# michaelfeil/skyjo_rl

Measured on AMD Instinct MI355X. Metric: env-steps/sec (whole node) at 65 536 parallel 3-player games, higher is better.
Workload: dtype int8

## Files before the change

skyjo_rl_amd/csrc/skyjo_deal.h:

```cpp
#pragma once
#ifndef SKYJO_DEVICE_PARTS
#error "include skyjo_device.h"
#endif

__global__ void k_seed(SkParams P, const uint64_t *seeds, uint64_t base, int first, int count) {
  const int i = blockIdx.x * blockDim.x + threadIdx.x;
  if (i >= count) return;
  const int g = first + i;
  const uint64_t value = seeds ? seeds[i] : base + P.game_id0 + (uint64_t)g;
  const size_t G = (size_t)P.tiles * SK_TILE;
  P.seeds[g] = value;
  P.deals_consumed[g] = 0;
  for (int k = 0; k < SK_BANK; k++) P.spare_ready[(size_t)k * G + g] = 0;
  P.bank_head[g] = 0, P.busy[g] = 0, P.cancel[g] = 0, P.done_flag[g] = 0;
  if (P.rng_mode == SKYJO_RNG_MT19937) {
    uint32_t *mt = P.mt + (size_t)g * 624;
    uint32_t x = (uint32_t)(value + 1);
    mt[0] = x;
    for (int k = 1; k < 624; k++) {
      x = 1812433253u * (x ^ (x >> 30)) + (uint32_t)k;
      mt[k] = x;
    }
    P.mt_idx[g] = 0;
  }
// ... 385 lines not shown
      w |= (i < SK_NCARDS ? (uint32_t)((-2 + i / 10) & 0xff) : 0u) << (8 * j);
    }
    LW(pw + d) = w;
  }
#pragma unroll 1
  for (int seg = 0; seg < N + 2; seg++) {
    int base = pb, n = SK_NCARDS;
    if (seg == 1) {
      for (int p = 0; p < N; p++)
        for (int j = 0; j < 3; j++) LW((sk_pb(P.L, p) >> 2) + j) = LW(pw + 3 * p + j);
      for (int d = 0; d < (R + 3) / 4; d += 8) {
        uint32_t t[8];
#pragma unroll
        for (int k = 0; k < 8; k++) t[k] = LW(pw + 3 * N + d + k);
#pragma unroll
        for (int k = 0; k < 8; k++)
          if (d + k < (R + 3) / 4) LW(pw + d + k) = t[k];
      }
      n = R;
    } else if (seg >= 2) {
      const int p = seg - 2;
      for (int k = 0; k < 12; k++) LB(tmp + k) = (uint8_t)k, LB(sk_pb(P.L, p) + PB_VIS + k) = SKYJO_HAND_NONE;
      base = tmp, n = 12;
    }
    shuffle_lds(lp, base, n, r);
    if (seg >= 2) {
      const int p = seg - 2;
      int s0 = LB(tmp), s1 = LB(tmp + 1);
      const int blk = sk_pb(P.L, p);
      int c0 = LI(blk + PB_CARDS + s0), c1 = LI(blk + PB_CARDS + s1);
      LB(blk + PB_VIS + s0) = (uint8_t)c0, LB(blk + PB_VIS + s1) = (uint8_t)c1;
      LSH(blk + PB_SUM) = (int16_t)(c0 + c1);
      LB(blk + PB_HIDDEN) = 10;
      if (!P.L.indirect) LB(H_HIST + 2 + c0)++, LB(H_HIST + 2 + c1)++;
    }
  }
  for (int k = R; k < SK_NCARDS; k++) LB(pb + k) = 0;
  const int last = LI(pb + R - 1);
  LB(pb + R - 1) = 0;
  LB(pb + SK_NCARDS - 1) = (uint8_t)last;
  LB(H_HIST + 2 + last)++;
  int best = 0, bs = LSH(sk_pb(P.L, 0) + PB_SUM);
  for (int p = 1; p < N; p++) {
    int s = LSH(sk_pb(P.L, p) + PB_SUM);
    if (s > bs) bs = s, best = p;
  }
  LB(H_PHASE) = 0, LB(H_PLAYER) = (uint8_t)best, LB(H_FLAGS) = F_VALID, LB(H_STATUS) = SKYJO_ST_RESET;
  LB(H_NDRAW) = (uint8_t)(R - 1), LB(H_NDISC) = 1, LB(H_ROLE) = 0;
  LB(H_TOP) = (uint8_t)last, LB(H_HAND) = SKYJO_HAND_NONE;
  *(uint32_t *)(lp + LIDX(H_EPISODE)) = episode;
  refresh_minima(P, lp);
}

__device__ __forceinline__ bool deal_inline(const SkParams &P, uint8_t *lp, uint8_t *fp, int g, int tile, int lane, int head) {
  const uint32_t ep = P.deals_consumed[g];
  const int busy = P.busy[g];
  if (busy) {
    const bool cancelled = P.cancel[g] != 0;
    if (P.rng_mode == SKYJO_RNG_MT19937 && !cancelled) {
      const int w = wait_deal_done(P, g);
      if (w == SK_WAIT_TIMEOUT) {
        LB(H_FLAGS) = F_VALID | F_DONE, LB(H_STATUS) = SKYJO_ST_ERROR;
        for (int q = 0; q < P.L.N; q++) P.rewards[(size_t)g * P.L.N + q] = 0.0;
        return false;
      }
      P.cancel[g] = 1;
      if (w == SK_WAIT_OK) {
        load_spare(P, lp, busy - 1, tile, lane);
        bank_advance(P, lp, g, head, ep);
        return true;
      }
    }
    P.cancel[g] = 1;
  }
  if (P.rng_mode == SKYJO_RNG_MT19937) {
    MtStream<16> r;
    r.open(P.mt + (size_t)g * 624, P.mt_idx[g], fp);
    deal_into_lds(P, lp, r, ep);
    P.mt_idx[g] = r.close();
  } else {
    PhiloxStream r;
    r.open(P.seeds[g] + 1, ep, 0u, 0u);
    deal_into_lds(P, lp, r, ep);
  }
  LB(H_BANK) = (uint8_t)head;
  P.deals_consumed[g] = ep + 1;
  P.done[g] = 0;
  return true;
}

#define SK_SCAN_BLOCK 1024
__global__ __launch_bounds__(SK_SCAN_BLOCK) void k_scan(SkParams P, int list_sel) {
  __shared__ uint32_t wave_need[SK_SCAN_BLOCK / 64], block_first;
  const size_t G = (size_t)P.tiles * SK_TILE;
  const int lane = threadIdx.x & 63, wave = threadIdx.x >> 6;
  int32_t *list = P.deal_list + (size_t)list_sel * G;
  uint32_t *eps = P.deal_ep + (size_t)list_sel * G;
  for (int base = blockIdx.x * SK_SCAN_BLOCK; base < P.B; base += gridDim.x * SK_SCAN_BLOCK) {
    const int g = base + (int)threadIdx.x;
    bool need = false;
    int slot = 0, r = 0;
    uint32_t consumed = 0;
    if (g < P.B) {
      const uint8_t busy = P.busy[g];
      const int head = P.bank_head[g] % SK_BANK;
      consumed = P.deals_consumed[g];
      uint8_t ready[SK_BANK];
// ... 208 lines not shown
```

skyjo_rl_amd/csrc/skyjo_device.h:

```cpp
#pragma once
#include <hip/hip_runtime.h>
#include <stdint.h>

#include "../../include/skyjo_vec.h"
#include "skyjo_layout.h"
#include "skyjo_draw.h"

struct SkCounters {
  unsigned long long steps, episodes, illegal, resets, sum_len, reshuffles, iters, waits;
  double sum_score[SKYJO_MAX_PLAYERS];
  double sum_reward[SKYJO_MAX_PLAYERS];
  double sum_reward_sq[SKYJO_MAX_PLAYERS];
  double sum_refunded[SKYJO_MAX_PLAYERS];
};
#define SK_ERR_DEAL_TIMEOUT 1u
#ifndef SK_SCORE_EVERY
#define SK_SCORE_EVERY 32
#endif
#define SK_ACC_KINDS 4

#ifndef SK_BANK
#define SK_BANK 3
#endif

// ... 107 lines not shown

#define SK_DMA4(NT)                                                                                                     \
  asm volatile("s_mov_b32 %0, m0\n\ts_mov_b32 m0, %3\n\ts_nop 0\n\t"                                                    \
               "global_load_lds_dwordx4 %1, %2" NT "\n\tglobal_load_lds_dwordx4 %1, %2 offset:1024" NT "\n\t"           \
               "global_load_lds_dwordx4 %1, %2 offset:2048" NT "\n\tglobal_load_lds_dwordx4 %1, %2 offset:3072" NT "\n\t" \
               "s_mov_b32 m0, %0"                                                                                       \
               : "=&s"(keep)                                                                                            \
               : "v"(voff), "s"(base), "s"(lds)                                                                         \
               : "memory")
#define SK_DMA1(NT)                                                                                              \
  asm volatile("s_mov_b32 %0, m0\n\ts_mov_b32 m0, %3\n\ts_nop 0\n\tglobal_load_lds_dwordx4 %1, %2" NT "\n\ts_mov_b32 m0, %0" \
               : "=&s"(keep)                                                                                     \
               : "v"(voff), "s"(base), "s"(lds)                                                                  \
               : "memory")
template <bool NT>
__device__ __forceinline__ void dma_record(const uint8_t *base, uint32_t voff, uint32_t lds, int chunks) {
  uint32_t keep;
  int c = 0;
  for (; c + 4 <= chunks; c += 4) {
    if (NT) SK_DMA4(" nt");
    else SK_DMA4("");
    base += 4096, lds += 4096;
  }
  for (; c < chunks; c++) {
    if (NT) SK_DMA1(" nt");
    else SK_DMA1("");
    base += 1024, lds += 1024;
  }
}
#define SK_DMAB4(NT)                                                                                                        \
  asm volatile("s_mov_b32 %0, m0\n\ts_mov_b32 m0, %3\n\ts_nop 0\n\tglobal_load_lds_dwordx4 %1, %2" NT "\n\t"                \
               "s_add_u32 m0, m0, 0x3f0\n\ts_nop 0\n\tglobal_load_lds_dwordx4 %1, %2 offset:16" NT "\n\t"                   \
               "s_add_u32 m0, m0, 0x3f0\n\ts_nop 0\n\tglobal_load_lds_dwordx4 %1, %2 offset:32" NT "\n\t"                   \
               "s_add_u32 m0, m0, 0x3f0\n\ts_nop 0\n\tglobal_load_lds_dwordx4 %1, %2 offset:48" NT "\n\t"                   \
               "s_mov_b32 m0, %0"                                                                                           \
               : "=&s"(keep)                                                                                                \
               : "v"(voff), "s"(base), "s"(lds)                                                                             \
               : "memory", "scc")
template <bool NT>
__device__ __forceinline__ void dma_bank_record(const uint8_t *base, uint32_t voff, uint32_t lds, int chunks) {
  uint32_t keep;
  int c = 0;
  for (; c + 4 <= chunks; c += 4) {
    if (NT) SK_DMAB4(" nt");
    else SK_DMAB4("");
    base += 64, lds += 4096;
  }
  for (; c < chunks; c++) {
    if (NT) SK_DMA1(" nt");
    else SK_DMA1("");
    base += 16, lds += 1024;
  }
}
__device__ __forceinline__ void sk_vm_drain() { asm volatile("s_waitcnt vmcnt(0)" ::: "memory"); }

struct Stamps {
  unsigned long long t, acc[8];
};
#ifdef SK_STAMPS
#define STAMP_DECL Stamps st; st.t = __builtin_amdgcn_s_memtime(); for (int k_ = 0; k_ < 8; k_++) st.acc[k_] = 0
#define STAMP(i)                                                 \
  do {                                                           \
    __builtin_amdgcn_sched_barrier(0);                           \
    __builtin_amdgcn_s_waitcnt(0xc07f);  \
    unsigned long long st_n = __builtin_amdgcn_s_memtime();      \
    __builtin_amdgcn_s_waitcnt(0xc07f);                          \
    st.acc[i] += st_n - st.t;                                    \
    st.t = st_n;                                                 \
    __builtin_amdgcn_sched_barrier(0);                           \
  } while (0)
#define STAMP_STORE                                                        \
  do {                                                                     \
    if (lane == 0)                                                         \
      for (int k = 0; k < 8; k++) P.stamps[(size_t)tile * 8 + k] += st.acc[k]; \
  } while (0)
#else
#define STAMP_DECL Stamps st
#define STAMP(i)
#define STAMP_STORE
#endif
#ifdef SK_STAMPS_TOP
#define STAMP_N(n)
#define STAMP_T(t) STAMP(t)
#else
#define STAMP_N(n) STAMP(n)
#define STAMP_T(t)
#endif

#ifdef SK_TRACE
#define TRACE_DECL const unsigned long long trace_t0 = __builtin_amdgcn_s_memrealtime(), trace_c0 = __builtin_amdgcn_s_memtime(); unsigned long long trace_wait = 0, trace_w0 = 0
#define TRACE_WAIT_BEGIN trace_w0 = __builtin_amdgcn_s_memtime()
#define TRACE_WAIT_END trace_wait += __builtin_amdgcn_s_memtime() - trace_w0
#define TRACE_STORE(kind, tag, lane_, block_)                                                                    \
  do {                                                                                                           \
    if ((lane_) == 0) {                                                                                          \
      unsigned long long *tr = P.stamps + (((size_t)(2 * (kind) + ((tag) & 1u)) * P.tiles + (block_)) * 8);     \
      tr[0] = __builtin_amdgcn_s_getreg(63492);                                       \
      tr[1] = __builtin_amdgcn_s_getreg(63508);                                               \
      tr[2] = trace_t0, tr[3] = __builtin_amdgcn_s_memrealtime(), tr[4] = (tag);                                 \
      tr[5] = __builtin_amdgcn_s_memtime() - trace_c0;  \
      tr[6] = trace_wait;                        \
    }                                                                                                            \
  } while (0)
#else
#define TRACE_DECL
#define TRACE_WAIT_BEGIN
#define TRACE_WAIT_END
#define TRACE_STORE(kind, tag, lane_, block_)
#endif

#define SKYJO_DEVICE_PARTS 1
#include "skyjo_rng.h"
#include "skyjo_transition.h"
#include "skyjo_record.h"
#include "skyjo_step.h"
#include "skyjo_deal.h"
#include "skyjo_cycle.h"
#include "skyjo_callers.h"
```

skyjo_rl_amd/csrc/skyjo_record.h:

```cpp
#pragma once
#ifndef SKYJO_DEVICE_PARTS
#error "include skyjo_device.h"
#endif

template <bool INDIRECT>
__device__ __forceinline__ void emit_record(const SkParams &P, uint8_t *lp, const HdrRegs &h, const ObsRegs &ob, int action,
                                            uint8_t *out, uint4 *held = nullptr, const uint4 *pre_a = nullptr, uint32_t pre_b = 0) {
  const int phase = h.w0 & 0xff;
  const uint32_t q0 = ob.q0, q1 = ob.q1, q2 = ob.q2;
  const uint32_t act24 = ((uint32_t)action & 0xffu) << 24;
  uint32_t m[8];
  {
    const uint32_t pm = phase ? 0xffffffffu : 0u;
    m[0] = ob.nz0 & pm, m[1] = ob.nz1 & pm, m[2] = ob.nz2 & pm, m[3] = ob.hd0 & pm, m[4] = ob.hd1 & pm, m[5] = ob.hd2 & pm;
    m[6] = (phase ? 0u : 0x0101u) | (((h.w0 >> 8) & 0xffu) << 16) | ((uint32_t)phase << 24);
    m[7] = (((h.w0 >> 16) & F_DONE) ? 1u : 0u) | ((h.w0 >> 24) << 8) | ((h.w2 & 0xffffu) << 16);
  }
  const uint4 a = pre_a ? *pre_a : LQ(1);
  const uint32_t s8 = (pre_a ? pre_b : (uint32_t)LB(32)) | ((h.w1 >> 24) << 8) | ((h.w2 >> 24) << 16);
  if (INDIRECT) {
    uint4 *o = (uint4 *)out;
    uint4 b;
    b.x = s8 | (q0 << 24), b.y = (q0 >> 8) | (q1 << 24), b.z = (q1 >> 8) | (q2 << 24), b.w = (q2 >> 8) | act24;
    if (held) {
// ... 45 lines not shown
    uint4 v[6];
#pragma unroll
    for (int k = 0; k < 6; k++)
      if (c + k < n) v[k] = LQ(c + k);
#pragma unroll
    for (int k = 0; k < 6; k++)
      if (c + k < n) d[c + k] = v[k];
  }
}

__device__ __forceinline__ void bank_advance(const SkParams &P, uint8_t *lp, int g, int head, uint32_t dc) {
  const uint8_t nh = (uint8_t)((head + 1) % SK_BANK);
  P.bank_head[g] = nh;
  LB(H_BANK) = nh;
  P.deals_consumed[g] = dc + 1;
  P.done[g] = 0;
}

__device__ __forceinline__ bool consume_spare(const SkParams &P, uint8_t *lp, int tile, int lane, int g, int head) {
  const size_t G = (size_t)P.tiles * SK_TILE;
  const uint8_t ready = P.spare_ready[(size_t)head * G + g];
  const uint32_t dc = P.deals_consumed[g];
  if (!ready) return false;
  load_spare(P, lp, head, tile, lane);
  P.spare_ready[(size_t)head * G + g] = 0;
  bank_advance(P, lp, g, head, dc);
  return true;
}

struct SpareRegs {
  uint32_t dc;
  int head;
  uint8_t ready;
};
__device__ __forceinline__ void spare_issue(const SkParams &P, uint8_t *lp, uint32_t lds_tile, int tile, int lane, int g, SpareRegs &r) {
  const size_t G = (size_t)P.tiles * SK_TILE;
  r.head = LB(H_BANK) % SK_BANK;
  r.ready = P.spare_ready[(size_t)r.head * G + g];
  r.dc = P.deals_consumed[g];
  const uint32_t voff = (uint32_t)(bank_rec16(P, r.head, g) * 16);
  asm volatile("s_waitcnt lgkmcnt(0)" ::: "memory");
  dma_bank_record<false>((const uint8_t *)P.spare, voff, lds_tile, P.L.chunks);
}
__device__ __forceinline__ bool spare_commit(const SkParams &P, uint8_t *lp, int g, const SpareRegs &r) {
  sk_vm_drain();
  if (!r.ready) return false;
  P.spare_ready[(size_t)r.head * (size_t)P.tiles * SK_TILE + g] = 0;
  bank_advance(P, lp, g, r.head, r.dc);
  return true;
}

__device__ __forceinline__ constexpr int sk_stage_stride(int rec_bytes) { return ((rec_bytes >> 2) & 7) == 0 ? rec_bytes + 16 : rec_bytes; }

__device__ __forceinline__ bool deal_inline(const SkParams &P, uint8_t *lp, uint8_t *fp, int g, int tile, int lane, int head);
```

skyjo_rl_amd/csrc/skyjo_step.h:

```cpp
#pragma once
#ifndef SKYJO_DEVICE_PARTS
#error "include skyjo_device.h"
#endif

__device__ __forceinline__ void sk_publish_deals(const SkParams &P, int g) {
  const size_t G = (size_t)P.tiles * SK_TILE;
  const int b = P.busy[g];
  if (b) {
    const uint32_t tag = P.plan_tag[g];
    const uint32_t f = __hip_atomic_load(&P.done_flag[g], __ATOMIC_RELAXED, __HIP_MEMORY_SCOPE_AGENT);
    if ((f & 0x7fffffffu) == tag) {
      SK_FENCE_ACQUIRE(P);
      if (!P.cancel[g] && f == tag) P.spare_ready[(size_t)(b - 1) * G + g] = 1;
      P.busy[g] = 0, P.cancel[g] = 0;
    }
  }
}
__device__ __forceinline__ void sk_plan_deals(const SkParams &P, int g, int lane) {
  const size_t G = (size_t)P.tiles * SK_TILE;
  bool need = false, empty = false;
  if (g < P.B) {
    const uint8_t busy = P.busy[g];
    const int head = P.bank_head[g] % SK_BANK;
    const uint32_t consumed = P.deals_consumed[g];
// ... 32 lines not shown
__device__ __forceinline__ void sk_export_raw(const SkParams &P, uint8_t *lp, int g, uint8_t *o) {
  for (int c = 0; c < P.L.chunks; c++) ((uint4 *)o)[c] = LQ(c);
  double *d = (double *)(o + P.L.state_bytes);
  for (int p = 0; p < P.L.N; p++) d[p] = P.rewards[(size_t)g * P.L.N + p], d[P.L.N + p] = P.scores[(size_t)g * P.L.N + p];
  uint32_t *m = (uint32_t *)(d + 2 * P.L.N);
  m[0] = P.rng_mode == SKYJO_RNG_MT19937 ? (uint32_t)P.mt_idx[g] : 0u;
  m[1] = P.done[g];
}

__device__ __forceinline__ uint32_t sk_next_tag(uint32_t t) {
  t = (t + 1u) & 0x7fffffffu;
  return t ? t : 1u;
}
template <bool INDIRECT, bool POLICY, int NP, bool PLANAR = false>
__device__ __forceinline__ void step_body(const SkParams &Pin, const int tile, const int lane, uint32_t *lds_raw, const int32_t *actions,
                                          uint8_t *rec_out, int32_t *act_out, int iters, uint64_t policy_seed, uint64_t iter0,
                                          double *end_rew_out, uint8_t *end_out, uint8_t *raw_out, int raw_stride, const int cycle_len = 0,
                                          const bool defer_ok = true) {
  SkParams P = Pin;
  TRACE_DECL;
  if (NP > 0) P.L = sk_make_layout(NP, INDIRECT ? 1 : 0);
  const int g = tile * SK_TILE + lane;
  const uint32_t lds_tile = (uint32_t)(uintptr_t)(__attribute__((address_space(3))) uint32_t *)lds_raw;
  uint8_t *lp = (uint8_t *)lds_raw + lane * 16;
  uint8_t *stg = (uint8_t *)lds_raw + P.L.chunks * 1024;
  uint8_t *fp = stg + lane * 4;
  const int stg_bytes = (INDIRECT || PLANAR) ? 4096 : SK_TILE * (P.L.rec_bytes + 16);
  uint8_t *ap = stg + stg_bytes + lane * 8;
  constexpr bool DEFER = POLICY && NP > 0 && NP < 8;
  constexpr bool REGACC = NP > 0 && NP < 8;
  constexpr int NACC = REGACC ? SK_ACC_KINDS * NP : 1;
  double racc_store[NACC];
#pragma unroll
  for (int k = 0; k < NACC; k++) racc_store[k] = 0.0;
  double *racc = REGACC ? racc_store : nullptr;
  uint8_t *pendp = DEFER && defer_ok ? stg + stg_bytes + (REGACC ? 0 : SK_ACC_KINDS * P.L.N * 512) + lane * 16 : nullptr;
  int pend_fin = -1;
  if (!REGACC)
    for (int k = 0; k < SK_ACC_KINDS * P.L.N; k++) ACC(k) = 0.0;
  STAMP_DECL;
  if (!POLICY) tile_load(P, P.state, tile, lane, lp);
  else dma_record<true>((const uint8_t *)P.state, (uint32_t)((((size_t)tile * P.L.chunks) * SK_TILE + lane) * 16), lds_tile, P.L.chunks);
  if (P.ov_flags & 1u) sk_publish_deals(P, g);
  sk_vm_drain();
  HdrRegs h;
  HDR_LOAD(h);
  STAMP(0);
  const bool valid = ((h.w0 >> 16) & F_VALID) != 0;
  LaneCounters cnt;
  uint32_t r0 = 0, r1 = 0, r2 = 0, r3 = 0;
  const uint64_t gid = P.game_id0 + (uint64_t)g;
  ObsRegs ob;
  if (valid) obs_load(P, lp, (h.w0 >> 8) & 0xff, ob);
  for (int it = 0; it < iters; it++) {
    const uint64_t iter = iter0 + (uint64_t)it;
    if (POLICY && (it == 0 || (iter & 3) == 0)) {
      philox4x32_10((uint32_t)(iter >> 2), (uint32_t)gid, (uint32_t)(gid >> 32), 0x504F4C00u, (uint32_t)policy_seed,
                    (uint32_t)(policy_seed >> 32), r0, r1, r2, r3);
      for (int k = (int)(iter & 3); k > 0; k--) {
        const uint32_t t = r0;
        r0 = r1, r1 = r2, r2 = r3, r3 = t;
      }
    }
    STAMP_T(3);
    const uint32_t word = r0;
    if (POLICY) {
      r0 = r1, r1 = r2, r2 = r3, r3 = word;
    }
    int a = -1;
    if (valid) {
      const bool over = ((h.w0 >> 16) & F_DONE) != 0;
      if (!POLICY) a = actions[g];
      const bool skip = !POLICY && a == SKYJO_ACTION_SKIP;
      const bool acted = !over && !skip;
      SpareRegs sp;
      const bool resetting = over && P.auto_reset && !skip;
      if (resetting) spare_issue(P, lp, lds_tile, tile, lane, g, sp);
      STAMP_T(4);
      if (!over && !skip) {
        const uint32_t v0 = ob.q0, v1 = ob.q1, v2 = ob.q2;
        STAMP_N(2);
        const uint4 row_pre = LQ(sk_pb(P.L, (h.w0 >> 8) & 0xff) >> 4);
        asm volatile("" ::: "memory");
        if (POLICY) a = policy_pick(h.w0 & 0xff, ob, word);
#ifndef SK_STAMPS_FINE
        STAMP_N(3);
#endif
        apply_action<INDIRECT, NP, POLICY>(P, lp, fp, ap, h, v0, v1, v2, a, g, cnt, st, pendp, pend_fin, row_pre, racc);
#ifdef SK_STAMPS_FINE
        STAMP(6);
#else
        STAMP(5);
#endif
      } else if (!skip) {
        a = -1;
        if (P.auto_reset) {
          bool dealt = true;
          if (!spare_commit(P, lp, g, sp)) {
            dealt = deal_inline(P, lp, fp, g, tile, lane, sp.head);
            cnt.waits++;
          }
          HDR_LOAD(h);
          if (SK_OFTEN(dealt)) {
            h.w0 = (h.w0 & 0x00ffffffu) | ((uint32_t)SKYJO_ST_RESET << 24);
            cnt.resets++;
          }
        } else {
          h.w0 = (h.w0 & 0x00ffffffu) | ((uint32_t)SKYJO_ST_NOOP_DONE << 24);
        }
        STAMP(1);
      } else {
        a = -1;
      }
      if (!POLICY && acted && (unsigned)a >= (unsigned)SKYJO_NUM_ACTIONS) a = -2;
      if (!POLICY && end_out) {
        const bool end = acted && ((h.w0 >> 16) & F_DONE) != 0;
        end_out[g] = end ? 1 : 0;
        for (int q = 0; q < P.L.N; q++) end_rew_out[(size_t)g * P.L.N + q] = end ? P.rewards[(size_t)g * P.L.N + q] : 0.0;
      }
      const uint4 rec_a = LQ(1);
      const uint32_t rec_b = LB(32);
      const uint4 rec_row = LQ((sk_pb(P.L, (h.w0 >> 8) & 0xff) + PB_VIS) >> 4);
      asm volatile("" ::: "memory");
      obs_from_row(rec_row, ob);
      if (rec_out) {
        if (INDIRECT) {
          uint4 rr[4];
          emit_record<INDIRECT>(P, lp, h, ob, a, nullptr, rr, &rec_a, rec_b);
          if (PLANAR) {
            typedef uint32_t u32x4_t __attribute__((ext_vector_type(4)));
            uint8_t *blk = rec_out + ((size_t)it * P.tiles + (size_t)tile) * (SK_TILE * 64) + lane * 16;
#pragma unroll
            for (int p = 0; p < 4; p++) __builtin_nontemporal_store((u32x4_t){rr[p].x, rr[p].y, rr[p].z, rr[p].w}, (u32x4_t *)(blk + p * 1024));
          } else {
#pragma unroll
            for (int p = 0; p < 4; p++) *(uint4 *)(stg + lane * 64 + ((p + (lane >> 1)) & 3) * 16) = rr[p];
          }
        } else if (PLANAR) {
          constexpr int PIECES = NP > 0 ? (((19 + 12 * NP + 3) & ~3) + 32 + 15) / 16 : 1;
          uint32_t wbuf[4 * PIECES];
#pragma unroll
          for (int k = 0; k < 4 * PIECES; k++) wbuf[k] = 0u;
          emit_record<INDIRECT>(P, lp, h, ob, a, (uint8_t *)wbuf, nullptr, &rec_a, rec_b);
          typedef uint32_t u32x4_t __attribute__((ext_vector_type(4)));
          uint8_t *blk = rec_out + ((size_t)it * P.tiles + (size_t)tile) * (SK_TILE * 16 * PIECES) + lane * 16;
#pragma unroll
          for (int p = 0; p < PIECES; p++)
            __builtin_nontemporal_store((u32x4_t){wbuf[4 * p], wbuf[4 * p + 1], wbuf[4 * p + 2], wbuf[4 * p + 3]}, (u32x4_t *)(blk + p * 1024));
        } else {
          emit_record<INDIRECT>(P, lp, h, ob, a, stg + lane * sk_stage_stride(P.L.rec_bytes), nullptr, &rec_a, rec_b);
        }
      }
      if (act_out) __builtin_nontemporal_store(a, &act_out[(size_t)it * P.B + g]);
#ifdef SK_STAMPS_FINE
      STAMP(7);
#else
      STAMP(6);
#endif
    }
    if (DEFER && ((it & (SK_SCORE_EVERY - 1)) == SK_SCORE_EVERY - 1 || it == iters - 1)) {
      if (SK_RARE(__any(pend_fin >= 0))) {
        if (pend_fin >= 0) {
          finish_game_fixed<(NP > 0 && NP < 8) ? NP : 1>(P, pendp, 1024, ap, g, pend_fin, racc);
          pend_fin = -1;
        }
      }
    }
    if (!INDIRECT && !PLANAR && rec_out) {
      typedef uint32_t u32x4_t __attribute__((ext_vector_type(4)));
      const int pieces = P.L.rec_bytes >> 4, stride = sk_stage_stride(P.L.rec_bytes);
      uint8_t *blk = rec_out + ((size_t)it * P.B + (size_t)tile * SK_TILE) * (size_t)P.L.rec_bytes;
      const int live = P.B - tile * SK_TILE;
      for (int q0 = lane; q0 < pieces * SK_TILE; q0 += 4 * SK_TILE) {
        uint4 v[4];
#pragma unroll
        for (int j = 0; j < 4; j++) {
          const int q = q0 + j * SK_TILE, r = q / pieces, p = q - r * pieces;
          if (q < pieces * SK_TILE) v[j] = *(const uint4 *)(stg + r * stride + p * 16);
        }
        if (SK_OFTEN(live >= SK_TILE)) {
#pragma unroll
          for (int j = 0; j < 4; j++) {
            const int q = q0 + j * SK_TILE;
            if (q0 - lane + j * SK_TILE < pieces * SK_TILE)
              __builtin_nontemporal_store((u32x4_t){v[j].x, v[j].y, v[j].z, v[j].w}, (u32x4_t *)(blk + (size_t)q * 16));
          }
        } else {
#pragma unroll
          for (int j = 0; j < 4; j++) {
            const int q = q0 + j * SK_TILE, r = q / pieces;
            if (q < pieces * SK_TILE && r < live)
              __builtin_nontemporal_store((u32x4_t){v[j].x, v[j].y, v[j].z, v[j].w}, (u32x4_t *)(blk + (size_t)q * 16));
          }
        }
      }
    }
    if (INDIRECT && !PLANAR && rec_out) {
      typedef uint32_t u32x4_t __attribute__((ext_vector_type(4)));
      uint8_t *blk = rec_out + ((size_t)it * P.B + (size_t)tile * SK_TILE) * 64;
      const int live = P.B - tile * SK_TILE;
      uint4 v[4];
#pragma unroll
      for (int j = 0; j < 4; j++) {
        const int r = 16 * j + (lane >> 2), p = lane & 3;
        v[j] = *(const uint4 *)(stg + r * 64 + ((p + (r >> 1)) & 3) * 16);
      }
      if (SK_OFTEN(live >= SK_TILE)) {
#pragma unroll
        for (int j = 0; j < 4; j++)
          __builtin_nontemporal_store((u32x4_t){v[j].x, v[j].y, v[j].z, v[j].w}, (u32x4_t *)(blk + j * 1024 + lane * 16));
      } else {
#pragma unroll
        for (int j = 0; j < 4; j++)
          if (16 * j + (lane >> 2) < live)
            __builtin_nontemporal_store((u32x4_t){v[j].x, v[j].y, v[j].z, v[j].w}, (u32x4_t *)(blk + j * 1024 + lane * 16));
      }
    }
    STAMP_T(2);
    if (POLICY && cycle_len && it + 1 < iters && (it + 1) % cycle_len == 0) {
      if (P.busy[g]) (void)wait_deal_done(P, g);
      sk_publish_deals(P, g);
      sk_plan_deals(P, g, lane);
      P.plan_new_tag = sk_next_tag(P.plan_new_tag);
      TRACE_WAIT_BEGIN;
      __syncthreads();
      TRACE_WAIT_END;
    }
  }
  HDR_FLUSH(h);
  tile_store_nt(P, P.state, tile, lane, lp);
  if (!POLICY && raw_out && valid) sk_export_raw(P, lp, g, raw_out + (size_t)g * raw_stride);
  if (P.ov_flags & 2u) {
    if (P.ov_flags & 1u) {
      if (P.busy[g]) (void)wait_deal_done(P, g);
      sk_publish_deals(P, g);
    }
    sk_plan_deals(P, g, lane);
  }
  if (!POLICY) {
    sk_error_to_host(P, lane);
    if (P.host_seq) {
      __threadfence_system();
      if (lane == 0) __hip_atomic_store(&P.health_host[3], P.host_seq, __ATOMIC_RELEASE, __HIP_MEMORY_SCOPE_SYSTEM);
    }
  }
  uint32_t v[7] = {cnt.steps, cnt.episodes, cnt.illegal, cnt.resets, cnt.sum_len, cnt.reshuffles, cnt.waits};
#pragma unroll
  for (int k = 0; k < 7; k++)
    for (int off = 32; off > 0; off >>= 1) v[k] += __shfl_down(v[k], off, 64);
  if (lane == 0) {
    unsigned long long *c = P.tile_counters + (size_t)tile * 8;
#pragma unroll
    for (int k = 0; k < 7; k++) c[k] += v[k];
  }
  if (__any(cnt.episodes | cnt.illegal)) {
    double mine = 0.0;
    if (REGACC) {
#pragma unroll
      for (int k = 0; k < NACC; k++) {
        double x = racc_store[k];
        for (int off = 32; off > 0; off >>= 1) x += __shfl_down(x, off, 64);
        x = __shfl(x, 0, 64);
        mine = lane == k ? x : mine;
      }
    } else {
      for (int k = 0; k < SK_ACC_KINDS * P.L.N; k++) {
        double x = ACC(k);
        for (int off = 32; off > 0; off >>= 1) x += __shfl_down(x, off, 64);
        x = __shfl(x, 0, 64);
        mine = lane == k ? x : mine;
      }
    }
    if (lane < SK_ACC_KINDS * P.L.N)
      P.acc_tile[(size_t)tile * SK_ACC_KINDS * SKYJO_MAX_PLAYERS + (lane / P.L.N) * SKYJO_MAX_PLAYERS + lane % P.L.N] += mine;
  }
  STAMP(7);
  STAMP_STORE;
  TRACE_STORE(0, (uint32_t)(iter0 / (uint64_t)(iters > 0 ? iters : 1)), lane, tile);
}

template <bool INDIRECT, bool POLICY, int NP, bool PLANAR = false>
// ... 71 lines not shown
```

skyjo_rl_amd/csrc/skyjo_transition.h:

```cpp
#pragma once
#ifndef SKYJO_DEVICE_PARTS
#error "include skyjo_device.h"
#endif

__device__ __forceinline__ void refresh_minima(const SkParams &P, uint8_t *lp) {
  int ms = LSH(sk_pb(P.L, 0) + PB_SUM), mh = LB(sk_pb(P.L, 0) + PB_HIDDEN);
  for (int q = 1; q < P.L.N; q++) {
    int s = LSH(sk_pb(P.L, q) + PB_SUM), h = LB(sk_pb(P.L, q) + PB_HIDDEN);
    ms = s < ms ? s : ms, mh = h < mh ? h : mh;
  }
  LB(H_MINSUM) = (uint8_t)(int8_t)(ms < 127 ? ms : 127);
  LB(H_MINHID) = (uint8_t)mh;
}

template <class Rng>
__device__ __forceinline__ void reshuffle_discard(const SkParams &P, uint8_t *lp, Rng &r) {
  const int n = LB(H_NDISC), role = LB(H_ROLE), pb = P.L.off_pile;
  const int reg = role ? 0 : 1;
  for (int i = n - 1; i >= 1; i--) {
    int j = (int)rng_interval(r, (uint32_t)i);
    int ai = pb + pile_addr(reg, i), aj = pb + pile_addr(reg, j);
    uint8_t t = LB(ai);
    LB(ai) = LB(aj), LB(aj) = t;
  }
// ... 1 lines not shown
  int last = LI(pb + pile_addr(reg, n - 1));
  LB(pb + pile_addr(reg ^ 1, 0)) = (uint8_t)last;
  LB(H_NDRAW) = (uint8_t)(n - 1), LB(H_NDISC) = 1, LB(H_ROLE) = (uint8_t)(role ^ 1);
  LB(H_TOP) = (uint8_t)last;
  int rs = LB(H_RESH);
  LB(H_RESH) = (uint8_t)(rs < 255 ? rs + 1 : 255);
}

#define SK_WAIT_OK 0
#define SK_WAIT_GAVE_UP 1
#define SK_WAIT_TIMEOUT 2
__device__ __forceinline__ int wait_deal_done(const SkParams &P, int g) {
  uint32_t f = 0;
  const uint32_t tag = P.plan_tag[g];
  for (int spin = 0; spin < (1 << P.spin_log2); spin++) {
    f = __hip_atomic_load(&P.done_flag[g], __ATOMIC_RELAXED, __HIP_MEMORY_SCOPE_AGENT);
    if ((f & 0x7fffffffu) == tag) break;
    __builtin_amdgcn_s_sleep(32);
  }
  if ((f & 0x7fffffffu) != tag) {
    atomicOr(P.dev_error, SK_ERR_DEAL_TIMEOUT);
    return SK_WAIT_TIMEOUT;
  }
  SK_FENCE_ACQUIRE(P);
  return (f >> 31) != 0 ? SK_WAIT_GAVE_UP : SK_WAIT_OK;
}

__device__ __forceinline__ uint32_t mt_untwist_y(const uint32_t *mt, int i) {
  uint32_t t = mt[i] ^ mt[i + 397 >= 624 ? i + 397 - 624 : i + 397];
  const uint32_t odd = t >> 31;
  t ^= odd ? 0x9908b0dfu : 0u;
  return (t << 1) | odd;
}
__device__ __forceinline__ void mt_untwist(uint32_t *mt, int from, int to) {
  for (int i = to; i != from;) {
    const int nx = i == 624 ? 0 : i;
    i = nx == 0 ? 623 : nx - 1;
    const uint32_t y = mt_untwist_y(mt, i);
    const int ip1 = i == 623 ? 0 : i + 1;
    mt[ip1] = (mt[ip1] & 0x80000000u) | (y & 0x7fffffffu);
    mt[i] = y & 0x80000000u;
  }
}

__device__ __forceinline__ int mt_rollback(const SkParams &P, uint32_t *mt, int g, int slot, int packed) {
  const size_t G = (size_t)P.tiles * SK_TILE;
  const int snap = P.mt_idx[(size_t)(1 + slot) * G + g];
  int from = (snap & 0xffff) + (snap >> 16), to = (packed & 0xffff) + (packed >> 16);
  from = from >= 624 ? from - 624 : from, to = to >= 624 ? to - 624 : to;
  mt_untwist(mt, from, to);
  return snap;
}

__device__ __forceinline__ void reshuffle_dispatch(const SkParams &P, uint8_t *lp, uint8_t *fp, int g) {
  if (P.rng_mode == SKYJO_RNG_MT19937) {
    const size_t G = (size_t)P.tiles * SK_TILE;
    uint32_t *mt = P.mt + (size_t)g * 624;
    const int head = LB(H_BANK) % SK_BANK;
    const int busy = P.busy[g];
    const bool inflight = busy && !P.cancel[g];
    bool undo_inflight = false;
    if (inflight) {
      const int w = wait_deal_done(P, g);
      if (w == SK_WAIT_TIMEOUT) {
        LB(H_FLAGS) |= F_DONE, LB(H_STATUS) = SKYJO_ST_ERROR, LB(H_NDRAW) = 1;
        P.done[g] = 1;
        for (int q = 0; q < P.L.N; q++) P.rewards[(size_t)g * P.L.N + q] = 0.0;
        return;
      }
      undo_inflight = w == SK_WAIT_OK;
      P.cancel[g] = 1;
    }
    int packed = P.mt_idx[g];
    if (undo_inflight) packed = mt_rollback(P, mt, g, busy - 1, packed);
    for (int k = SK_BANK - 1; k >= 0; k--) {
      const int slot = (head + k) % SK_BANK;
      if (P.spare_ready[(size_t)slot * G + g]) {
        packed = mt_rollback(P, mt, g, slot, packed);
        P.spare_ready[(size_t)slot * G + g] = 0;
      }
    }
    MtStream<16> r;
    r.open(mt, packed, fp);
    reshuffle_discard(P, lp, r);
    P.mt_idx[g] = r.close();
  } else {
    PhiloxStream r;
    r.open(P.seeds[g] + 1, *(uint32_t *)(lp + LIDX(H_EPISODE)), LB(H_RESH), 1u);
    reshuffle_discard(P, lp, r);
  }
}

#define ACC(k) (*(double *)(ap + ((k) << 9)))
__device__ __forceinline__ void acc_add(uint8_t *ap, int k, double v) {
  __hip_atomic_fetch_add(&ACC(k), v, __ATOMIC_RELAXED, __HIP_MEMORY_SCOPE_WAVEFRONT);
}
__device__ __forceinline__ void acc_episode(uint8_t *ap, int N, int p, double score, double reward, int refunded) {
  acc_add(ap, p, score), acc_add(ap, N + p, reward), acc_add(ap, 2 * N + p, reward * reward);
  if (refunded) acc_add(ap, 3 * N + p, (double)refunded);
}

__device__ __forceinline__ void finish_game(const SkParams &P, uint8_t *lp, uint8_t *fp, uint8_t *ap, int g,
                                            int finisher) {
  const int N = P.L.N;
  double *sc = P.scores + (size_t)g * N, *rw = P.rewards + (size_t)g * N;
  int mn = 0, fs = 0;
  for (int p = 0; p < N; p++) {
    int s = 0;
// ... 93 lines not shown
  uint32_t *w = (uint32_t *)(lp + LIDX(b & ~3));
  const uint32_t d = (uint32_t)delta << ((b & 3) * 8);
  __hip_atomic_fetch_add(w, d, __ATOMIC_RELAXED, __HIP_MEMORY_SCOPE_WAVEFRONT);
}
__device__ __forceinline__ uint32_t swar_nonzero01(uint32_t x) {
  return ((((x & 0x7f7f7f7fu) + 0x7f7f7f7fu) | x) & 0x80808080u) >> 7;
}
__device__ __forceinline__ uint32_t pack12(uint32_t a, uint32_t b, uint32_t c) {
  return ((a * 0x00204081u >> 21) & 0xfu) | (((b * 0x00204081u >> 21) & 0xfu) << 4) |
         (((c * 0x00204081u >> 21) & 0xfu) << 8);
}

struct ObsRegs {
  uint32_t q0, q1, q2, nz0, nz1, nz2, hd0, hd1, hd2;
};
__device__ __forceinline__ void obs_from_row(const uint4 &row, ObsRegs &o) {
  o.q0 = row.x, o.q1 = row.y, o.q2 = row.z;
  o.nz0 = swar_nonzero01(o.q0 ^ 0xf2f2f2f2u);
  o.nz1 = swar_nonzero01(o.q1 ^ 0xf2f2f2f2u);
  o.nz2 = swar_nonzero01(o.q2 ^ 0xf2f2f2f2u);
  o.hd0 = swar_nonzero01(o.q0 ^ 0x0f0f0f0fu) ^ 0x01010101u;
  o.hd1 = swar_nonzero01(o.q1 ^ 0x0f0f0f0fu) ^ 0x01010101u;
  o.hd2 = swar_nonzero01(o.q2 ^ 0x0f0f0f0fu) ^ 0x01010101u;
}
__device__ __forceinline__ void obs_load(const SkParams &P, uint8_t *lp, int q, ObsRegs &o) {
  const uint4 row = LQ((sk_pb(P.L, q) + PB_VIS) >> 4);
  obs_from_row(row, o);
}

__device__ __forceinline__ int policy_pick(int phase, const ObsRegs &o, uint32_t word) {
  if (phase == 0) return 24 + (int)__umulhi(word, 2u);
  uint32_t legal = pack12(o.nz0, o.nz1, o.nz2) | (pack12(o.hd0, o.hd1, o.hd2) << 12);
  const int n = __popc(legal);
  if (n == 0) return 24;
  int k = (int)__umulhi(word, (uint32_t)n), pos = 0;
  int c = __popc(legal & 0xfffu);
  if (k >= c) k -= c, pos = 12, legal >>= 12;
  c = __popc(legal & 0x3fu);
  if (k >= c) k -= c, pos += 6, legal >>= 6;
  c = __popc(legal & 0x7u);
  if (k >= c) k -= c, pos += 3, legal >>= 3;
  c = (int)(legal & 1u);
  if (k >= c) {
    k -= c, pos += 1;
    c = (int)((legal >> 1) & 1u);
    if (k >= c) pos += 1;
  }
  return pos;
}

template <bool INDIRECT, int NP, bool TRUSTED>
__device__ __forceinline__ void apply_action(const SkParams &P, uint8_t *lp, uint8_t *fp, uint8_t *ap, HdrRegs &h, uint32_t v0,
                                             uint32_t v1, uint32_t v2, int a, int g, LaneCounters &cnt, Stamps &st,
                                             uint8_t *pendp, int &pend_fin, const uint4 &row_pre, double *racc = nullptr) {
  const int N = P.L.N;
  const int phase = h.w0 & 0xff, p = (h.w0 >> 8) & 0xff;
  const int blk = sk_pb(P.L, p), cardb = blk + PB_CARDS, visb = blk + PB_VIS, pb = P.L.off_pile;
  const unsigned ua = (unsigned)a;
  int slot = 0, sv = 0;
  bool legal;
  if (ua < 24u) {
    slot = a < 12 ? a : a - 12;
    sv = byte3(v0, v1, v2, slot);
    legal = phase == 1 && (TRUSTED || (a < 12 ? sv != SKYJO_REFUNDED : sv == SKYJO_HAND_NONE));
  } else {
    legal = (TRUSTED || ua <= 25u) && phase == 0;
  }
  if (!legal) {
    double *rw = P.rewards + (size_t)g * N;
    for (int q = 0; q < N; q++) rw[q] = q == p ? P.illegal_reward : 0.0;
    if (NP > 0 && racc) {
#pragma unroll
      for (int q = 0; q < (NP > 0 ? NP : 1); q++)
        racc[NP + q] += q == p ? P.illegal_reward : 0.0, racc[2 * NP + q] += q == p ? P.illegal_reward * P.illegal_reward : 0.0;
    } else {
      acc_add(ap, N + p, P.illegal_reward), acc_add(ap, 2 * N + p, P.illegal_reward * P.illegal_reward);
    }
    h.w0 = (h.w0 & 0x0000ffffu) | ((((h.w0 >> 16) & 0xffu) | F_DONE) << 16) | ((uint32_t)SKYJO_ST_ILLEGAL << 24);
    P.done[g] = 1;
    cnt.illegal++;
    return;
  }
  const int eplen = (int)(h.w2 & 0xffffu) + 1;
  h.w2 = (h.w2 & 0xffff0000u) | (uint32_t)eplen;
  h.w0 &= 0x00ffffffu;
  cnt.steps++;
  if (phase == 0) {
    const int role = (h.w1 >> 16) & 1;
    int nd = h.w1 & 0xff;
    const int ns = (h.w1 >> 8) & 0xff;
    const int hidden_p = (int)((row_pre.w >> 16) & 0xffu);
    int pile_top = LI(pb + pile_addr(role, nd > 0 ? nd - 1 : 0));
    const int disc_top = LI(pb + pile_addr(role ^ 1, ns > 0 ? ns - 1 : 0));
    const int disc_below = LI(pb + pile_addr(role ^ 1, ns > 1 ? ns - 2 : 0));

    if (hidden_p == 0) {
      h.w0 |= (uint32_t)(F_TERMINATED | F_DONE) << 16;
      LB(H_FINISHER) = (uint8_t)p;
      if (NP > 0 && NP < 8) {
        constexpr int NQ = (NP > 0 && NP < 8) ? NP : 1;
        P.done[g] = 1;
        if (pendp) {
#pragma unroll
          for (int q = 0; q < NQ; q++) *(uint4 *)(pendp + q * 1024) = LQ(sk_pb(P.L, q) >> 4);
          pend_fin = p;
        } else {
          finish_game_fixed<NQ>(P, lp + (P.L.off_players >> 4) * 1024, 2048, ap, g, p, racc);
        }
      } else {
        finish_game(P, lp, fp, ap, g, p);
      }
      cnt.episodes++;
      cnt.sum_len += eplen;
#ifdef SK_STAMPS_FINE
      STAMP(3);
#endif
      return;
    }
    const bool from_pile = a == 24;
    if (from_pile && nd == 0) {
      HDR_FLUSH(h);
      reshuffle_dispatch(P, lp, fp, g);
      HDR_LOAD(h);
      cnt.reshuffles++;
      nd = h.w1 & 0xff;
      pile_top = LI(pb + pile_addr((h.w1 >> 16) & 1, nd - 1));
    }
    int hand;
    if (from_pile) {
      hand = pile_top;
      h.w1 = (h.w1 & 0xffffff00u) | (uint32_t)(nd - 1);
    } else {
      hand = disc_top;
      hist_add(lp, hand, -1);
      const int top = ns > 1 ? disc_below : -3;
      h.w1 = (h.w1 & 0x00ff00ffu) | ((uint32_t)(ns - 1) << 8) | (((uint32_t)top & 0xffu) << 24);
    }
    h.w2 = (h.w2 & 0x00ffffffu) | (((uint32_t)hand & 0xffu) << 24);
    h.w0 = (h.w0 & 0xffffff00u) | 1u;
#ifdef SK_STAMPS_FINE
    STAMP(3);
#endif
    return;
  }
  STAMP_N(4);
  const int hand = (int)(int8_t)(h.w2 >> 24);
  const int reg = ((h.w1 >> 16) & 1) ^ 1;
  int ns = (h.w1 >> 8) & 0xff;
  const uint4 row = row_pre;
  const uint32_t c0 = row.x, c1 = row.y, c2 = row.z;
  int sum = (int)(int16_t)(row.w & 0xffffu), hid = (int)((row.w >> 16) & 0xffu), refunded = (int)(row.w >> 24);
  int oms = 1 << 20, omh = 1 << 20;
  for (int q = 0; q < N; q++) {
    const uint32_t cq = LW((sk_pb(P.L, q) + PB_SUM) >> 2);
    const int s = (int)(int16_t)(cq & 0xffffu), hq = (int)((cq >> 16) & 0xffu);
    oms = (q != p && s < oms) ? s : oms, omh = (q != p && hq < omh) ? hq : omh;
  }
#ifdef SK_STAMPS_FINE
  STAMP(5);
#endif
  const bool swap = a < 12, was_hidden = sv == SKYJO_HAND_NONE;
  const int under = byte3(c0, c1, c2, slot);
  const int shown = swap ? hand : under, gone = swap ? under : hand;
  LB(pb + pile_addr(reg, ns)) = (uint8_t)gone;
  ns++;
  hist_add(lp, gone, 1);
  LB(cardb + slot) = (uint8_t)shown;
  LB(visb + slot) = (uint8_t)shown;
  put3(v0, v1, v2, slot, shown);
  sum += shown - (was_hidden ? 0 : under);
  hid -= was_hidden ? 1 : 0;
  if (!INDIRECT) {
    if (!was_hidden) hist_add(lp, under, -1);
    hist_add(lp, shown, 1);
  }
// ... 39 lines not shown
```

Measured before the change: 47.54 billion.

## Prefetch banked spare deals into an LDS pool ahead of game resets

Adds a small per-tile LDS pool of 12 entries. Once a game's next-turn state shows it is about to end, the kernel starts async global-to-LDS DMA of that game's next banked spare deal plus its ready flag and deal counter. On reset, a pool-served game copies the prefetched record into its LDS state instead of issuing and committing a synchronous spare load. Reshuffles and inline deals invalidate the pool and drain outstanding loads. This adds vmcnt waits, extra ballot and readlane loops, and pool bookkeeping to every iteration, plus optional reset-timing instrumentation.

```diff
diff --git a/skyjo_rl_amd/csrc/skyjo_deal.h b/skyjo_rl_amd/csrc/skyjo_deal.h
--- a/skyjo_rl_amd/csrc/skyjo_deal.h
+++ b/skyjo_rl_amd/csrc/skyjo_deal.h
@@ -461,7 +461,11 @@
   refresh_minima(P, lp);
 }
 
-__device__ __forceinline__ bool deal_inline(const SkParams &P, uint8_t *lp, uint8_t *fp, int g, int tile, int lane, int head) {
+__device__ __forceinline__ bool deal_inline(const SkParams &P, uint8_t *lp, uint8_t *fp, int g, int tile, int lane, int head, uint32_t *pool_drop) {
+  if (pool_drop) {
+    sk_vm_drain();
+    *pool_drop = ~0u;
+  }
   const uint32_t ep = P.deals_consumed[g];
   const int busy = P.busy[g];
   if (busy) {
diff --git a/skyjo_rl_amd/csrc/skyjo_device.h b/skyjo_rl_amd/csrc/skyjo_device.h
--- a/skyjo_rl_amd/csrc/skyjo_device.h
+++ b/skyjo_rl_amd/csrc/skyjo_device.h
@@ -183,12 +183,67 @@
     base += 16, lds += 1024;
   }
 }
+__device__ __forceinline__ void dma_bank_entry(const uint8_t *base, uint32_t voff, uint32_t lds) {
+  uint32_t keep;
+  SK_DMA1("");
+}
+__device__ __forceinline__ void dma_entry_words(const void *addr, uint32_t lds) {
+  uint32_t keep;
+  asm volatile("s_mov_b32 %0, m0\n\ts_mov_b32 m0, %2\n\ts_nop 0\n\tglobal_load_lds_dword %1, off\n\ts_mov_b32 m0, %0"
+               : "=&s"(keep)
+               : "v"(addr), "s"(lds)
+               : "memory");
+}
 __device__ __forceinline__ void sk_vm_drain() { asm volatile("s_waitcnt vmcnt(0)" ::: "memory"); }
 
 struct Stamps {
   unsigned long long t, acc[8];
 };
-#ifdef SK_STAMPS
+#if defined(SK_STAMPS) && defined(SK_STAMPS_RESET)
+#define STAMP_DECL Stamps st; st.t = 0; for (int k_ = 0; k_ < 8; k_++) st.acc[k_] = 0
+#define STAMP(i)
+#define RS_NOW(v)                                   \
+  do {                                              \
+    __builtin_amdgcn_sched_barrier(0);              \
+    __builtin_amdgcn_s_waitcnt(0xc07f);             \
+    v = __builtin_amdgcn_s_memtime();               \
+    __builtin_amdgcn_s_waitcnt(0xc07f);             \
+    __builtin_amdgcn_sched_barrier(0);              \
+  } while (0)
+#define RS_ITER_BEGIN(any_reset)  \
+  unsigned long long rs_t0;       \
+  const bool rs_any = (any_reset); \
+  RS_NOW(rs_t0)
+#define RS_ITER_END                                    \
+  do {                                                 \
+    unsigned long long rs_n;                           \
+    RS_NOW(rs_n);                                      \
+    st.acc[0]++;                                       \
+    if (rs_any) st.acc[1]++, st.acc[2] += rs_n - rs_t0; \
+    else st.acc[3] += rs_n - rs_t0;                    \
+  } while (0)
+#define RS_BEGIN(v) unsigned long long v; RS_NOW(v)
+#define RS_REQ_END(v, slot)     \
+  do {                          \
+    unsigned long long rs_n;    \
+    RS_NOW(rs_n);               \
+    st.acc[slot] += rs_n - v;   \
+  } while (0)
+#define RS_COMMIT_END(v)                                                                         \
+  do {                                                                                           \
+    unsigned long long rs_n;                                                                     \
+    RS_NOW(rs_n);                                                                                \
+    if (lane == __ffsll((long long)__ballot(true)) - 1) st.acc[5] += rs_n - v;  \
+  } while (0)
+#define RS_HANDOVER(from_pool) st.acc[7] += 1ull + ((from_pool) ? 1ull << 32 : 0ull)
+#define STAMP_STORE                                                                        \
+  do {                                                                                     \
+    for (int off = 32; off > 0; off >>= 1)                                                 \
+      st.acc[5] += __shfl_down(st.acc[5], off, 64), st.acc[7] += __shfl_down(st.acc[7], off, 64); \
+    if (lane == 0)                                                                         \
+      for (int k = 0; k < 8; k++) P.stamps[(size_t)tile * 8 + k] += st.acc[k];             \
+  } while (0)
+#elif defined(SK_STAMPS)
 #define STAMP_DECL Stamps st; st.t = __builtin_amdgcn_s_memtime(); for (int k_ = 0; k_ < 8; k_++) st.acc[k_] = 0
 #define STAMP(i)                                                 \
   do {                                                           \
@@ -209,6 +264,14 @@
 #define STAMP_DECL Stamps st
 #define STAMP(i)
 #define STAMP_STORE
+#endif
+#if !(defined(SK_STAMPS) && defined(SK_STAMPS_RESET))
+#define RS_ITER_BEGIN(any_reset)
+#define RS_ITER_END
+#define RS_BEGIN(v)
+#define RS_REQ_END(v, slot)
+#define RS_COMMIT_END(v)
+#define RS_HANDOVER(from_pool)
 #endif
 #ifdef SK_STAMPS_TOP
 #define STAMP_N(n)
diff --git a/skyjo_rl_amd/csrc/skyjo_record.h b/skyjo_rl_amd/csrc/skyjo_record.h
--- a/skyjo_rl_amd/csrc/skyjo_record.h
+++ b/skyjo_rl_amd/csrc/skyjo_record.h
@@ -121,4 +121,5 @@
 
 __device__ __forceinline__ constexpr int sk_stage_stride(int rec_bytes) { return ((rec_bytes >> 2) & 7) == 0 ? rec_bytes + 16 : rec_bytes; }
 
-__device__ __forceinline__ bool deal_inline(const SkParams &P, uint8_t *lp, uint8_t *fp, int g, int tile, int lane, int head);
+__device__ __forceinline__ bool deal_inline(const SkParams &P, uint8_t *lp, uint8_t *fp, int g, int tile, int lane, int head,
+                                            uint32_t *pool_drop = nullptr);
diff --git a/skyjo_rl_amd/csrc/skyjo_step.h b/skyjo_rl_amd/csrc/skyjo_step.h
--- a/skyjo_rl_amd/csrc/skyjo_step.h
+++ b/skyjo_rl_amd/csrc/skyjo_step.h
@@ -108,6 +108,12 @@
   const uint64_t gid = P.game_id0 + (uint64_t)g;
   ObsRegs ob;
   if (valid) obs_load(P, lp, (h.w0 >> 8) & 0xff, ob);
+  constexpr bool POOL = POLICY && PLANAR && NP > 0;
+  constexpr uint32_t PE_N = 12;
+  const uint32_t pe_bytes = (uint32_t)P.L.chunks * 16u + 16u;
+  uint32_t pool = 0;
+  uint32_t pool_used = 0;
+  const bool pool_on = POOL && P.auto_reset && __all(valid);
   for (int it = 0; it < iters; it++) {
     const uint64_t iter = iter0 + (uint64_t)it;
     if (POLICY && (it == 0 || (iter & 3) == 0)) {
@@ -119,11 +125,43 @@
       }
     }
     STAMP_T(3);
+    RS_ITER_BEGIN(__any(valid && ((h.w0 >> 16) & F_DONE) != 0 && P.auto_reset));
     const uint32_t word = r0;
+    bool served = false;
+    if (POOL && pool_on) {
+      const bool have = pool != 0 && ((h.w0 >> 16) & F_DONE) != 0;
+      if (__any(have)) {
+        RS_BEGIN(rs_a0);
+        if (rec_out && __all(!have || (((uint32_t)it - (pool >> 8)) & 0xffffffu) >= 3u)) asm volatile("s_waitcnt vmcnt(8)" ::: "memory");
+        else sk_vm_drain();
+        int head = 0;
+        uint32_t dc = 0;
+        if (have) {
+          const uint8_t *tl = stg + ((pool & 0xffu) - 1u) * pe_bytes + P.L.chunks * 16;
+          dc = *(const uint32_t *)(tl + 4);
+          served = ((*(const uint32_t *)tl >> ((g & 3) * 8)) & 0xffu) != 0;
+          head = LB(H_BANK) % SK_BANK;
+        }
+        const unsigned long long sm = __ballot(served);
+        for (unsigned long long m = __ballot(have); m; m &= m - 1) {
+          const int l = __ffsll((long long)m) - 1;
+          const uint32_t e = ((uint32_t)__builtin_amdgcn_readlane((int)pool, l) & 0xffu) - 1u;
+          pool_used &= ~(1u << e);
+          if (((sm >> l) & 1ull) && lane < P.L.chunks) *(uint4 *)((uint8_t *)lds_raw + lane * 1024 + l * 16) = *(const uint4 *)(stg + e * pe_bytes + lane * 16);
+        }
+        if (have) pool = 0;
+        if (served) {
+          P.spare_ready[(size_t)head * ((size_t)P.tiles * SK_TILE) + g] = 0;
+          bank_advance(P, lp, g, head, dc);
+        }
+        RS_COMMIT_END(rs_a0);
+      }
+    }
     if (POLICY) {
       r0 = r1, r1 = r2, r2 = r3, r3 = word;
     }
     int a = -1;
+    bool pool_want = false;
     if (valid) {
       const bool over = ((h.w0 >> 16) & F_DONE) != 0;
       if (!POLICY) a = actions[g];
@@ -131,7 +169,9 @@
       const bool acted = !over && !skip;
       SpareRegs sp;
       const bool resetting = over && P.auto_reset && !skip;
-      if (resetting) spare_issue(P, lp, lds_tile, tile, lane, g, sp);
+      RS_BEGIN(rs_q0);
+      if (resetting && !(POOL && served)) spare_issue(P, lp, lds_tile, tile, lane, g, sp);
+      RS_REQ_END(rs_q0, rs_any ? 4 : 6);
       STAMP_T(4);
       if (!over && !skip) {
         const uint32_t v0 = ob.q0, v1 = ob.q1, v2 = ob.q2;
@@ -142,7 +182,7 @@
 #ifndef SK_STAMPS_FINE
         STAMP_N(3);
 #endif
-        apply_action<INDIRECT, NP, POLICY>(P, lp, fp, ap, h, v0, v1, v2, a, g, cnt, st, pendp, pend_fin, row_pre, racc);
+        apply_action<INDIRECT, NP, POLICY>(P, lp, fp, ap, h, v0, v1, v2, a, g, cnt, st, pendp, pend_fin, row_pre, racc, POOL ? &pool : nullptr);
 #ifdef SK_STAMPS_FINE
         STAMP(6);
 #else
@@ -152,8 +192,9 @@
         a = -1;
         if (P.auto_reset) {
           bool dealt = true;
-          if (!spare_commit(P, lp, g, sp)) {
-            dealt = deal_inline(P, lp, fp, g, tile, lane, sp.head);
+          RS_BEGIN(rs_c0);
+          if (!(POOL && served) && !spare_commit(P, lp, g, sp)) {
+            dealt = deal_inline(P, lp, fp, g, tile, lane, sp.head, POOL ? &pool : nullptr);
             cnt.waits++;
           }
           HDR_LOAD(h);
@@ -161,6 +202,8 @@
             h.w0 = (h.w0 & 0x00ffffffu) | ((uint32_t)SKYJO_ST_RESET << 24);
             cnt.resets++;
           }
+          RS_COMMIT_END(rs_c0);
+          RS_HANDOVER(POOL && served);
         } else {
           h.w0 = (h.w0 & 0x00ffffffu) | ((uint32_t)SKYJO_ST_NOOP_DONE << 24);
         }
@@ -179,6 +222,7 @@
       const uint4 rec_row = LQ((sk_pb(P.L, (h.w0 >> 8) & 0xff) + PB_VIS) >> 4);
       asm volatile("" ::: "memory");
       obs_from_row(rec_row, ob);
+      if (POOL) pool_want = ((rec_a.x >> 8) & 0xffu) == 0 && ((h.w0 >> 16) & F_DONE) == 0;
       if (rec_out) {
         if (INDIRECT) {
           uint4 rr[4];
@@ -214,6 +258,31 @@
       STAMP(6);
 #endif
     }
+    if (POOL && pool_on) {
+      if (SK_RARE(__any(pool == ~0u))) pool = 0, pool_used = 0;
+      pool_want = pool_want && pool == 0;
+      unsigned long long wm = __ballot(pool_want);
+      if (wm) {
+        RS_BEGIN(rs_b0);
+        const uint32_t hb = pool_want ? (uint32_t)LB(H_BANK) : 0u;
+        asm volatile("s_waitcnt lgkmcnt(0)" ::: "memory");
+        const size_t G = (size_t)P.tiles * SK_TILE;
+        for (; wm; wm &= wm - 1) {
+          const uint32_t fr = ~pool_used & ((1u << PE_N) - 1u);
+          if (!fr) break;
+          const int l = __ffsll((long long)wm) - 1, gl = tile * SK_TILE + l;
+          const uint32_t e = (uint32_t)__builtin_amdgcn_readfirstlane(__ffs((int)fr) - 1), ent = lds_tile + (uint32_t)P.L.chunks * 1024u + e * pe_bytes;
+          const int head = (int)((uint32_t)__builtin_amdgcn_readlane((int)hb, l) % SK_BANK);
+          pool_used |= 1u << e;
+          if (lane < P.L.chunks) dma_bank_entry((const uint8_t *)P.spare, (uint32_t)(bank_rec16(P, head, gl) * 16) + (uint32_t)lane * 16u, ent);
+          if (lane < 2)
+            dma_entry_words(lane == 0 ? (const void *)(P.spare_ready + (((size_t)head * G + (size_t)gl) & ~(size_t)3)) : (const void *)(P.deals_consumed + gl),
+                            ent + (uint32_t)P.L.chunks * 16u);
+          if (lane == l) pool = (e + 1u) | ((uint32_t)it << 8);
+        }
+        RS_REQ_END(rs_b0, 4);
+      }
+    }
     if (DEFER && ((it & (SK_SCORE_EVERY - 1)) == SK_SCORE_EVERY - 1 || it == iters - 1)) {
       if (SK_RARE(__any(pend_fin >= 0))) {
         if (pend_fin >= 0) {
@@ -273,6 +342,7 @@
       }
     }
     STAMP_T(2);
+    RS_ITER_END;
     if (POLICY && cycle_len && it + 1 < iters && (it + 1) % cycle_len == 0) {
       if (P.busy[g]) (void)wait_deal_done(P, g);
       sk_publish_deals(P, g);
@@ -283,6 +353,7 @@
       TRACE_WAIT_END;
     }
   }
+  if (POOL && pool_on) sk_vm_drain();
   HDR_FLUSH(h);
   tile_store_nt(P, P.state, tile, lane, lp);
   if (!POLICY && raw_out && valid) sk_export_raw(P, lp, g, raw_out + (size_t)g * raw_stride);
diff --git a/skyjo_rl_amd/csrc/skyjo_transition.h b/skyjo_rl_amd/csrc/skyjo_transition.h
--- a/skyjo_rl_amd/csrc/skyjo_transition.h
+++ b/skyjo_rl_amd/csrc/skyjo_transition.h
@@ -77,8 +77,12 @@
   return snap;
 }
 
-__device__ __forceinline__ void reshuffle_dispatch(const SkParams &P, uint8_t *lp, uint8_t *fp, int g) {
+__device__ __forceinline__ void reshuffle_dispatch(const SkParams &P, uint8_t *lp, uint8_t *fp, int g, uint32_t *pool_drop = nullptr) {
   if (P.rng_mode == SKYJO_RNG_MT19937) {
+    if (pool_drop) {
+      sk_vm_drain();
+      *pool_drop = ~0u;
+    }
     const size_t G = (size_t)P.tiles * SK_TILE;
     uint32_t *mt = P.mt + (size_t)g * 624;
     const int head = LB(H_BANK) % SK_BANK;
@@ -278,7 +282,8 @@
 template <bool INDIRECT, int NP, bool TRUSTED>
 __device__ __forceinline__ void apply_action(const SkParams &P, uint8_t *lp, uint8_t *fp, uint8_t *ap, HdrRegs &h, uint32_t v0,
                                              uint32_t v1, uint32_t v2, int a, int g, LaneCounters &cnt, Stamps &st,
-                                             uint8_t *pendp, int &pend_fin, const uint4 &row_pre, double *racc = nullptr) {
+                                             uint8_t *pendp, int &pend_fin, const uint4 &row_pre, double *racc = nullptr,
+                                             uint32_t *pool_drop = nullptr) {
   const int N = P.L.N;
   const int phase = h.w0 & 0xff, p = (h.w0 >> 8) & 0xff;
   const int blk = sk_pb(P.L, p), cardb = blk + PB_CARDS, visb = blk + PB_VIS, pb = P.L.off_pile;
@@ -346,7 +351,7 @@
     const bool from_pile = a == 24;
     if (from_pile && nd == 0) {
       HDR_FLUSH(h);
-      reshuffle_dispatch(P, lp, fp, g);
+      reshuffle_dispatch(P, lp, fp, g, pool_drop);
       HDR_LOAD(h);
       cnt.reshuffles++;
       nd = h.w1 & 0xff;
```

Result: slower. 38.17 billion (-19.7%).
